# injun-baek/Video-Depth-Normal-v2

Hardware: AMD Instinct MI355X
Metric: depth frames/sec at 518x518, ViT-L (higher is better)
Workload: dtype f16x3; 1 GPU; DepthAnythingV2(vitl) batch=8 518x518 streams/GPU, memory bank full (S=6); replicas per GPU; lanes=2, precision=f16x3, ranks=1, backend=none, attention_pv_products=1

## Files before the change

video-depth-normal-v2_amd/csrc/attn.hip:

```cpp
#include "common.hpp"
#include <cstdlib>
#include <type_traits>
#include <utility>

namespace {

__device__ __forceinline__ bool lane_hi() { return (threadIdx.x & 32) != 0; }
__device__ __forceinline__ int perm23(int i) {
  return (i & ~12) | ((i & 4) << 1) | ((i & 8) >> 1);
}
__device__ __forceinline__ int acc_key(int reg, int h) {
  return (reg & 3) + 4 * ((reg >> 2) & 1) + 8 * h + 16 * (reg >> 3);
}

__device__ __forceinline__ float xhalf(float v) {
  const unsigned u = __builtin_bit_cast(unsigned, v);
  const auto r = __builtin_amdgcn_permlane32_swap(u, u, false, false);
  return __builtin_bit_cast(float, (lane_hi() ? r[0] : r[1]));
}

template <class F, int... J>
__device__ __forceinline__ void for_each_slot_impl(F& f, std::integer_sequence<int, J...>) {
  (f(std::integral_constant<int, J>{}), ...);
}
// ... 300 lines not shown
      for (int i = 0; i < 16; ++i) { o[0][i] *= alpha; o[1][i] *= alpha; }
    }
    if constexpr (VDN_ATTN_ABL & 2) asm volatile("s_waitcnt vmcnt(0) lgkmcnt(0)" ::: "memory");
    else stage_barrier();
  };

  stage_k(0, 0);
  if (nt > 1) stage_k(1, 1);
  stage_barrier();
  qk(0, s);
  stage_barrier();
  constexpr std::true_type Y{};
  constexpr std::false_type N{};
  if (nt == 1) {
    iter(0, N, N);
  } else {
    iter(0, N, Y);
    for (int t = 1; t + 1 < nt; ++t) iter(t, Y, Y);
    iter(nt - 1, Y, N);
  }
  pv((nt - 1) & 1, pf, pl);

  const float l_tot = l_run + __shfl_xor(l_run, 32);
  const float inv = 1.0f / l_tot;
  const int q = q0 + r;
  if (q < nq) {
    const int b = bh / H, hd = bh - b * H;
    const size_t oo = (((size_t)b * nq + q) * H + hd) * 64;
#pragma unroll
    for (int db = 0; db < 2; ++db)
#pragma unroll
      for (int g = 0; g < 4; ++g) {
        typename HT::V4 v, vl;
#pragma unroll
        for (int e = 0; e < 4; ++e) {
          const float x = o[db][4 * g + e] * inv;
          if (outl) {
            T a, b2;
            split_rtz(x, a, b2);
            v[e] = a;
            vl[e] = b2;
          } else {
            v[e] = (T)x;
          }
        }
        *(typename HT::V4*)(out + oo + db * 32 + 8 * g + 4 * h) = v;
        if (outl) *(typename HT::V4*)(outl + oo + db * 32 + 8 * g + 4 * h) = vl;
      }
  }
}

#include "attn2_kernel.hpp"

template <int DT, bool SPLIT, int NB >
__global__ __launch_bounds__(256) void temporal_attn_kernel(const typename Half<DT>::T* __restrict__ qkv,
                                                            typename Half<DT>::T* __restrict__ out,
                                                            const typename Half<DT>::T* __restrict__ qkv_lo,
                                                            typename Half<DT>::T* __restrict__ out_lo, int nseq,
                                                            int Tn, int D, int c, int heads, float scale_log2,
                                                            const float* __restrict__ rope_cs) {
  using HT = Half<DT>;
  using T = typename HT::T;
  using V8 = typename HT::V8;
  const int lane = threadIdx.x & 63;
  const int seq = blockIdx.x * 4 + (threadIdx.x >> 6);
  if (seq >= nseq) return;
  const int head = seq % heads;
  const int bd = seq / heads;
  const int d = bd % D, b = bd / D;
  const int dh = c / heads;
  const int r = lane & 31, h = lane >> 5;
  const size_t rs = (size_t)D * 3 * c;
  const size_t boff = ((size_t)b * Tn * D + d) * 3 * c + head * dh;
  const T* base = qkv + boff;
  const T* base_lo = SPLIT ? qkv_lo + boff : nullptr;
  const T* vb = base + 2 * c;
  const T* vb_lo = SPLIT ? base_lo + 2 * c : nullptr;
  const size_t ooff = ((size_t)b * Tn * D + d) * c + head * dh;
  T* ob = out + ooff;
  T* ob_lo = SPLIT ? out_lo + ooff : nullptr;
  const size_t os = (size_t)D * c;
  const int nks = (dh + 15) >> 4;
  const int neb = (dh + 31) >> 5;
  const int pk = perm23(r);

  for (int qb = 0; qb < NB; ++qb) {
    if (qb * 32 >= Tn) break;
    const int tq = qb * 32 + r;
    const int fq = tq < Tn ? tq : Tn - 1;
    f32x16 s[NB];
#pragma unroll
    for (int kb = 0; kb < NB; ++kb) {
#pragma unroll
      for (int i = 0; i < 16; ++i) s[kb][i] = 0.f;
      if (kb * 32 >= Tn) continue;
      const int tk = kb * 32 + pk;
      const int fk = tk < Tn ? tk : Tn - 1;
      for (int ks = 0; ks < nks; ++ks) {
        const int e0 = 16 * ks + 8 * h;
        V8 a, bq, al, bl;
#pragma unroll
        for (int j = 0; j < 8; ++j) { a[j] = (T)0.f; bq[j] = (T)0.f; al[j] = (T)0.f; bl[j] = (T)0.f; }
        if (e0 < dh) {
          bq = *(const V8*)(base + fq * rs + e0);
          a = *(const V8*)(base + fk * rs + c + e0);
          if constexpr (SPLIT) {
            bl = *(const V8*)(base_lo + fq * rs + e0);
            al = *(const V8*)(base_lo + fk * rs + c + e0);
          }
          if (rope_cs) {
            const size_t pair0 = (size_t)(head * dh + e0) >> 1;
            auto rot = [&](V8& hi, V8& lo, int frame) {
              const float* cs = rope_cs + ((size_t)frame * (c >> 1) + pair0) * 2;
#pragma unroll
              for (int j = 0; j < 8; j += 2) {
                const float x0 = (float)hi[j] + (SPLIT ? (float)lo[j] : 0.f), x1 = (float)hi[j + 1] + (SPLIT ? (float)lo[j + 1] : 0.f);
                const float cc = cs[j], ss = cs[j + 1];
                const float y0 = x0 * cc - x1 * ss, y1 = x0 * ss + x1 * cc;
                if constexpr (SPLIT) {
                  T h0, h1, l0, l1;
                  split2_rtz(y0, y1, h0, h1, l0, l1);
                  hi[j] = h0; hi[j + 1] = h1; lo[j] = l0; lo[j + 1] = l1;
                } else {
                  hi[j] = (T)y0; hi[j + 1] = (T)y1;
                }
              }
            };
            rot(bq, bl, fq);
            rot(a, al, fk);
          }
        }
        s[kb] = HT::mfma32(a, bq, s[kb]);
        if constexpr (SPLIT) {
          s[kb] = HT::mfma32(a, bl, s[kb]);
          s[kb] = HT::mfma32(al, bq, s[kb]);
        }
      }
    }
    float mx = -1e30f;
#pragma unroll
    for (int kb = 0; kb < NB; ++kb)
#pragma unroll
      for (int i = 0; i < 16; ++i) {
        float v = s[kb][i] * scale_log2;
        v = (kb * 32 + acc_key(i, h) < Tn) ? v : -INFINITY;
        s[kb][i] = v;
        mx = fmaxf(mx, v);
      }
    mx = fmaxf(mx, __shfl_xor(mx, 32));
    float ls = 0.f;
    V8 pf[NB][2], pl[NB][2];
#pragma unroll
    for (int kb = 0; kb < NB; ++kb)
#pragma unroll
      for (int i = 0; i < 16; ++i) {
        const float pv = __builtin_amdgcn_exp2f(s[kb][i] - mx);
        ls += pv;
        if constexpr (SPLIT) {
          T a2, b2;
          split_rtz(pv, a2, b2);
          pf[kb][i >> 3][i & 7] = a2;
          pl[kb][i >> 3][i & 7] = b2;
        } else {
          pf[kb][i >> 3][i & 7] = (T)pv;
        }
      }
    ls += __shfl_xor(ls, 32);
    const float inv = 1.0f / ls;

    for (int eb = 0; eb < neb; ++eb) {
      f32x16 o;
#pragma unroll
      for (int i = 0; i < 16; ++i) o[i] = 0.f;
      const int e = eb * 32 + r;
#pragma unroll
      for (int kb = 0; kb < NB; ++kb) {
        if (kb * 32 >= Tn) continue;
#pragma unroll
        for (int sp = 0; sp < 2; ++sp) {
          V8 a, al;
#pragma unroll
          for (int j = 0; j < 8; ++j) {
            const int key = kb * 32 + 16 * sp + 8 * h + j;
            const bool ok = key < Tn && e < dh;
            a[j] = ok ? vb[key * rs + e] : (T)0.f;
            if constexpr (SPLIT) al[j] = ok ? vb_lo[key * rs + e] : (T)0.f;
          }
          o = HT::mfma32(a, pf[kb][sp], o);
          if constexpr (SPLIT) {
            o = HT::mfma32(a, pl[kb][sp], o);
            o = HT::mfma32(al, pf[kb][sp], o);
          }
        }
      }
      if (tq < Tn) {
#pragma unroll
        for (int g = 0; g < 4; ++g) {
          const int e0 = eb * 32 + 8 * g + 4 * h;
          if (e0 < dh) {
            typename HT::V4 v, vl;
#pragma unroll
            for (int q = 0; q < 4; ++q) {
              const float x = o[4 * g + q] * inv;
              if constexpr (SPLIT) {
                T a2, b2;
                split_rtz(x, a2, b2);
                v[q] = a2;
                vl[q] = b2;
              } else {
                v[q] = (T)x;
              }
            }
            *(typename HT::V4*)(ob + tq * os + e0) = v;
            if constexpr (SPLIT) *(typename HT::V4*)(ob_lo + tq * os + e0) = vl;
          }
        }
      }
    }
  }
}

struct SlotTable { int s[32]; };

template <int DT, int CPL >
__global__ __launch_bounds__(256) void temporal_last_kernel(const float* __restrict__ pool, size_t slot_stride, SlotTable tab,
                                                            int T, int HW, int c,
                                                            const float* __restrict__ peq, const float* __restrict__ pek,
                                                            const float* __restrict__ pev, float scale,
                                                            typename Half<DT>::T* __restrict__ out,
                                                            typename Half<DT>::T* __restrict__ out_lo) {
  using Th = typename Half<DT>::T;
  const int lane = threadIdx.x & 63;
  const int px = blockIdx.x * 4 + (threadIdx.x >> 6);
  if (px >= HW) return;
  const int ch = lane * CPL;
  const size_t row = (size_t)px * 3 * c;
  float q[CPL];
  {
    const float* qn = pool + (size_t)tab.s[T - 1] * slot_stride + row + ch;
#pragma unroll
    for (int e = 0; e < CPL; ++e) q[e] = (qn[e] + peq[(size_t)(T - 1) * c + ch + e]) * scale;
  }
  float sc[32];
  float mx = -INFINITY;
#pragma unroll
  for (int t = 0; t < 32; ++t) {
    sc[t] = -INFINITY;
    if (t < T) {
      const float* kt = pool + (size_t)tab.s[t] * slot_stride + row + c + ch;
      const float* pk = pek + (size_t)t * c + ch;
      float d = 0.f;
#pragma unroll
      for (int e = 0; e < CPL; ++e) d = fmaf(q[e], kt[e] + pk[e], d);
      d += __shfl_xor(d, 1);
      d += __shfl_xor(d, 2);
      d += __shfl_xor(d, 4);
      sc[t] = d;
      mx = fmaxf(mx, d);
    }
  }
  float den = 0.f;
#pragma unroll
  for (int t = 0; t < 32; ++t) {
    sc[t] = t < T ? __expf(sc[t] - mx) : 0.f;
    den += sc[t];
  }
  const float inv = 1.0f / den;
  float o[CPL];
#pragma unroll
  for (int e = 0; e < CPL; ++e) o[e] = 0.f;
#pragma unroll
  for (int t = 0; t < 32; ++t) {
    if (t < T) {
      const float* vt = pool + (size_t)tab.s[t] * slot_stride + row + 2 * c + ch;
      const float* pv = pev + (size_t)t * c + ch;
      const float p = sc[t] * inv;
#pragma unroll
      for (int e = 0; e < CPL; ++e) o[e] = fmaf(p, vt[e] + pv[e], o[e]);
    }
  }
#pragma unroll
  for (int e = 0; e < CPL; ++e) store_half(out, out_lo, (size_t)px * c + ch + e, o[e]);
}

template <int DT>
int flash_launch(const void* Q, const void* K, const void* Vt, void* out, const void* Ql, const void* Kl, const void* Vtl,
                 void* outl, const void* Q8, const void* K8, void* out8, int out_kt, int B, int H, int nq, int nq_pad, int nk, int nk_pad,
                 float sl2, int pv, hipStream_t s) {
  using T = typename Half<DT>::T;
  const dim3 grid(((nq + 127) / 128) * B * H);
  const bool pv3 = pv == 3;
  const uint8_t* q8 = (const uint8_t*)Q8;
  const uint8_t* k8 = (const uint8_t*)K8;
  if ((out8 || out_kt || (Ql && !outl)) && !(Ql && !pv3 && q8 && k8 && DT == VDN_F16)) return VDN_EUNSUPPORTED;
  if (Ql && pv3)
    hipLaunchKernelGGL((flash_attn_kernel<DT, true, false, false>), grid, dim3(256), 65536, s, (const T*)Q, (const T*)K, (const T*)Vt,
                       (T*)out, (const T*)Ql, (const T*)Kl, (const T*)Vtl, (T*)outl, q8, k8, H, nq, nq_pad, nk, nk_pad, sl2);
  else if (Ql && q8 && k8 && DT == VDN_F16) {
    if constexpr (DT == VDN_F16) {
#ifndef VDN_ATTN2_NW
#define VDN_ATTN2_NW 4
#endif
      constexpr int NW = VDN_ATTN2_NW;
      const dim3 grid2(((nq + 32 * NW - 1) / (32 * NW)) * B * H);
      if (pv == 1)
        hipLaunchKernelGGL((flash_attn2_kernel<1, NW>), grid2, dim3(64 * NW), (VDN_ATTN_ABL & 32) ? 98304 : 65536, s, (const T*)Q, (const T*)K, (const T*)Vt, (T*)out,
                           (const T*)Kl, (const T*)Vtl, (T*)outl, q8, k8, H, nq, nq_pad, nk, nk_pad, sl2, (uint8_t*)out8, out_kt, B * nq);
      else
        hipLaunchKernelGGL((flash_attn2_kernel<2, NW>), grid2, dim3(64 * NW), (VDN_ATTN_ABL & 32) ? 98304 : 65536, s, (const T*)Q, (const T*)K, (const T*)Vt, (T*)out,
                           (const T*)Kl, (const T*)Vtl, (T*)outl, q8, k8, H, nq, nq_pad, nk, nk_pad, sl2, (uint8_t*)out8, out_kt, B * nq);
    }
  } else if (Ql)
    hipLaunchKernelGGL((flash_attn_kernel<DT, true, true, false>), grid, dim3(256), 65536, s, (const T*)Q, (const T*)K, (const T*)Vt,
                       (T*)out, (const T*)Ql, (const T*)Kl, (const T*)Vtl, (T*)outl, q8, k8, H, nq, nq_pad, nk, nk_pad, sl2);
  else
    hipLaunchKernelGGL((flash_attn_kernel<DT, false, false, false>), grid, dim3(256), 32768, s, (const T*)Q, (const T*)K, (const T*)Vt,
                       (T*)out, (const T*)nullptr, (const T*)nullptr, (const T*)nullptr, (T*)outl, q8, k8, H, nq, nq_pad, nk,
                       nk_pad, sl2);
  VDN_CHECK_LAUNCH();
  return VDN_OK;
}

template <int DT>
int temporal_launch(const void* qkv, void* out, const void* qkv_lo, void* out_lo, int nseq, int T, int D, int c, int heads,
                    float sl2, const float* rope_cs, hipStream_t s) {
  using TT = typename Half<DT>::T;
  const dim3 grid((nseq + 3) / 4);
#define VDN_TA(SP, NB_)                                                                                          \
  hipLaunchKernelGGL((temporal_attn_kernel<DT, SP, NB_>), grid, dim3(256), 0, s, (const TT*)qkv, (TT*)out,       \
                     (const TT*)(SP ? qkv_lo : nullptr), (TT*)(SP ? out_lo : nullptr), nseq, T, D, c, heads, sl2, rope_cs)
  if (qkv_lo) {
    if (T <= 32) VDN_TA(true, 1); else VDN_TA(true, 2);
  } else {
    if (T <= 32) VDN_TA(false, 1); else VDN_TA(false, 2);
  }
#undef VDN_TA
  VDN_CHECK_LAUNCH();
  return VDN_OK;
}

}

extern "C" int vdn_flash_attn(int dt, const void* Q, const void* K, const void* Vt, void* out, const void* Q_lo,
                              const void* K_lo, const void* Vt_lo, void* out_lo, const void* Q8, const void* K8, void* out8,
                              int out_kt, int B, int H, int nq, int nq_pad, int nk, int nk_pad, float scale, int pv_products,
                              vdn_stream stream) {
  if (!Q || !K || !Vt || !out || B <= 0 || H <= 0 || nq <= 0 || nk <= 0) return VDN_EINVAL;
  if (pv_products < 0 || pv_products > 3) return VDN_EINVAL;
  const int pv = pv_products ? pv_products : 1;
  if (nq_pad < nq || nk_pad < nk || (nk_pad & 63)) return VDN_EALIGN;
  if (((uintptr_t)Q | (uintptr_t)K | (uintptr_t)Vt | (uintptr_t)out) & 15) return VDN_EALIGN;
  const int nlo = (Q_lo != nullptr) + (K_lo != nullptr) + (Vt_lo != nullptr);
  if (nlo != 0 && nlo != 3) return VDN_EINVAL;
  if (nlo == 3 && !out_lo && !out8) return VDN_EINVAL;
  if (((uintptr_t)Q_lo | (uintptr_t)K_lo | (uintptr_t)Vt_lo | (uintptr_t)out_lo | (uintptr_t)Q8 | (uintptr_t)K8 | (uintptr_t)out8) & 15) return VDN_EALIGN;
  if ((Q8 == nullptr) != (K8 == nullptr) || (Q8 && (nlo != 3 || dt != VDN_F16))) return VDN_EINVAL;
  const float sl2 = scale * 1.44269504088896340736f;
  hipStream_t s = (hipStream_t)stream;
  if (dt == VDN_F16)
    return flash_launch<VDN_F16>(Q, K, Vt, out, Q_lo, K_lo, Vt_lo, out_lo, Q8, K8, out8, out_kt, B, H, nq, nq_pad, nk, nk_pad, sl2, pv, s);
  if (dt == VDN_BF16)
    return flash_launch<VDN_BF16>(Q, K, Vt, out, Q_lo, K_lo, Vt_lo, out_lo, nullptr, nullptr, out8, out_kt, B, H, nq, nq_pad, nk, nk_pad, sl2, pv, s);
  return VDN_EUNSUPPORTED;
}

extern "C" int vdn_temporal_attn(int dt, const void* qkv, void* out, const void* qkv_lo, void* out_lo, int Bv, int T,
                                 int D, int c, int heads, float scale, const float* rope_cs, vdn_stream stream) {
  if (!qkv || !out || Bv <= 0 || T <= 0 || T > 64 || D <= 0 || heads <= 0 || c % heads) return VDN_EINVAL;
  if ((qkv_lo == nullptr) != (out_lo == nullptr)) return VDN_EINVAL;
  const int dh = c / heads;
  if ((dh & 7) || dh > 256 || (c & 7)) return VDN_EALIGN;
  if (((uintptr_t)qkv | (uintptr_t)out | (uintptr_t)qkv_lo | (uintptr_t)out_lo) & 15) return VDN_EALIGN;
  const int nseq = Bv * D * heads;
  const float sl2 = scale * 1.44269504088896340736f;
  hipStream_t s = (hipStream_t)stream;
  return with_half(dt, [&](auto t) {
    return temporal_launch<decltype(t)::value>(qkv, out, qkv_lo, out_lo, nseq, T, D, c, heads, sl2, rope_cs, s);
  });
}

extern "C" int vdn_temporal_attn_last(int dt, const float* pool, size_t slot_stride, const int32_t* slots, int T, int HW,
                                      int c, const float* pe_q, const float* pe_k, const float* pe_v, float scale,
                                      void* out, void* out_lo, vdn_stream stream) {
  if (!pool || !slots || !pe_q || !pe_k || !pe_v || !out || T < 1 || T > 32 || HW <= 0) return VDN_EINVAL;
  if (slot_stride < (size_t)HW * 3 * c) return VDN_EINVAL;
  SlotTable tab;
  for (int t = 0; t < 32; ++t) {
    tab.s[t] = t < T ? slots[t] : 0;
    if (tab.s[t] < 0) return VDN_EINVAL;
  }
  if (c <= 0 || (c & 63) || c > 1024) return VDN_EUNSUPPORTED;
  hipStream_t s = (hipStream_t)stream;
  const dim3 grid((HW + 3) / 4), block(256);
#define VDN_TL(CPL_)                                                                                                     \
  hipLaunchKernelGGL((temporal_last_kernel<DT, CPL_>), grid, block, 0, s, pool, slot_stride, tab, T, HW, c, pe_q, pe_k, \
                     pe_v, scale, (typename Half<DT>::T*)out, (typename Half<DT>::T*)out_lo)
  return with_half(dt, [&](auto t) -> int {
    constexpr int DT = decltype(t)::value;
    switch (c) {
      case 64: VDN_TL(1); break;
      case 128: VDN_TL(2); break;
      case 192: VDN_TL(3); break;
      case 256: VDN_TL(4); break;
      case 384: VDN_TL(6); break;
      case 512: VDN_TL(8); break;
      case 768: VDN_TL(12); break;
      case 1024: VDN_TL(16); break;
      default: return VDN_EUNSUPPORTED;
    }
    VDN_CHECK_LAUNCH();
    return VDN_OK;
  });
#undef VDN_TL
}
```

video-depth-normal-v2_amd/csrc/attn2_kernel.hpp:

```cpp

template <int PV, int NW>
__global__ __launch_bounds__(64 * NW) __attribute__((amdgpu_waves_per_eu(2, 2))) void flash_attn2_kernel(
    const _Float16* __restrict__ Q, const _Float16* __restrict__ K, const _Float16* __restrict__ Vt, _Float16* __restrict__ out,
    const _Float16* __restrict__ Kl, const _Float16* __restrict__ Vtl, _Float16* __restrict__ outl, const uint8_t* __restrict__ Q8,
    const uint8_t* __restrict__ K8, int H, int nq, int nq_pad, int nk, int nk_pad, float scale_log2, uint8_t* __restrict__ out8,
    int out_kt, int out_rows) {
  using HT = Half<VDN_F16>;
  using T = _Float16;
  using V8 = typename HT::V8;
  constexpr int TILE = 8192;
  constexpr int NT = 4;
  extern __shared__ __attribute__((aligned(16))) char smem[];

  const int tid = threadIdx.x, lane = tid & 63;
  const int wave = __builtin_amdgcn_readfirstlane(tid >> 6);
  constexpr int QB = 32 * NW;
  constexpr int NPC = 8 / NW;
  const int nqb = (nq + QB - 1) / QB;
  const int logical = xcd_remap(blockIdx.x, gridDim.x);
  const int bh = logical / nqb;
  const int q0 = (logical - bh * nqb) * QB + wave * 32;
  const int r = lane & 31, h = lane >> 5;

  V8 qf[4];
  i32x8 q8h, q8l;
  {
    int q = q0 + r;
    q = q < nq ? q : nq - 1;
    const size_t qo = ((size_t)bh * nq_pad + q) * 64 + 8 * h;
#pragma unroll
    for (int ks = 0; ks < 4; ++ks) qf[ks] = *(const V8*)(Q + qo + 16 * ks);
    const uint8_t* q8 = Q8 + ((size_t)bh * nq_pad + q) * 128 + 32 * h;
    const u32x4 a0 = *(const u32x4*)q8, a1 = *(const u32x4*)(q8 + 16), b0 = *(const u32x4*)(q8 + 64), b1 = *(const u32x4*)(q8 + 80);
#pragma unroll
    for (int e = 0; e < 4; ++e) { q8h[e] = (int)a0[e]; q8h[4 + e] = (int)a1[e]; q8l[e] = (int)b0[e]; q8l[4 + e] = (int)b1[e]; }
  }

  const int lr = lane >> 3;
  const unsigned k_bytes = (unsigned)nk_pad * 64 * sizeof(T);
  const auto rsrc = [&](const void* base) {
    return __builtin_amdgcn_make_buffer_rsrc((void*)((const char*)base + (size_t)bh * k_bytes), 0, (int)k_bytes, 0x00020000);
  };
  const __amdgpu_buffer_rsrc_t rK = rsrc(K), rV = rsrc(Vt), rK8 = rsrc(K8), rVl = rsrc(Vtl);
  int koff[2], voff[2];
#pragma unroll
  for (int i = 0; i < NPC; ++i) {
    const int row = (wave + 4 * i) * 8 + lr;
    const int c = (lane & 7) ^ ((row >> 1) & 7);
    koff[i] = (row * 64 + c * 8) * (int)sizeof(T);
    voff[i] = (row * nk_pad + c * 8) * (int)sizeof(T);
  }
#define A2_BLDS16(rs, voffset, soffset, dst) \
  __builtin_amdgcn_raw_ptr_buffer_load_lds(rs, (__attribute__((address_space(3))) void*)(dst), 16, voffset, soffset, 0, 0)
  auto stage_k_piece = [&](int buf, int t, int i, bool second) {
    A2_BLDS16(second ? rK8 : rK, koff[i], t * (64 * 64 * (int)sizeof(T)), smem + buf * NT * TILE + (second ? 2 * TILE : 0) + (wave + 4 * i) * 1024);
  };
  auto stage_v_piece = [&](int buf, int t, int i, bool second) {
    A2_BLDS16(second ? rVl : rV, voff[i], t * (64 * (int)sizeof(T)), smem + buf * NT * TILE + TILE + (second ? 2 * TILE : 0) + (wave + 4 * i) * 1024);
  };

  const int k_base = perm23(r) * 128 + ((h ^ ((perm23(r) >> 1) & 7)) << 4);
  const int v_base = r * 128 + ((h ^ ((r >> 1) & 7)) << 4);
  const int k8_base = perm23(r) * 128 + (((2 * h) ^ ((perm23(r) >> 1) & 7)) << 4);
  auto k_addr = [&](int kb, int ks) { return kb * 4096 + (k_base ^ (ks << 5)); };
  auto v_addr = [&](int db, int c) { return db * 4096 + (v_base ^ (c << 5)); };
  auto k8_read = [&](const char* sK, int kb, int lo) {
    const char* p = sK + 2 * TILE + kb * 4096;
    const u32x4 a0 = *(const u32x4*)(p + (k8_base ^ ((4 * lo) << 4))), a1 = *(const u32x4*)(p + (k8_base ^ ((4 * lo + 1) << 4)));
    i32x8 v;
#pragma unroll
    for (int e = 0; e < 4; ++e) { v[e] = (int)a0[e]; v[4 + e] = (int)a1[e]; }
    return v;
  };
  auto cross_hl = [&](const i32x8& k8, f32x16 c) {
    return __builtin_amdgcn_mfma_scale_f32_32x32x64_f8f6f4(k8, q8l, c, 1, 1, 0, 127, 0, VDN_LO8_E8M0);
  };
  auto cross_lh = [&](const i32x8& k8l, f32x16 c) {
    return __builtin_amdgcn_mfma_scale_f32_32x32x64_f8f6f4(k8l, q8h, c, 1, 1, 0, VDN_LO8_E8M0, 0, 127);
  };

  f32x16 o[2], s[2][2];
  V8 pf[2][2][2];
#pragma unroll
  for (int i = 0; i < 16; ++i) { o[0][i] = 0.f; o[1][i] = 0.f; }
  float m_run = -1e30f, l_run = 0.f;
  constexpr float LAZY = 6.0f;
  const int nt = (nk + 63) >> 6;
  const f32x16 zero16 = {0.f, 0.f, 0.f, 0.f, 0.f, 0.f, 0.f, 0.f, 0.f, 0.f, 0.f, 0.f, 0.f, 0.f, 0.f, 0.f};

#if VDN_ATTN_ABL & 64
  unsigned long long stamp_sum[5] = {0, 0, 0, 0, 0}, stamp_last = 0;
#endif
#define A2_IC(n) std::integral_constant<int, n> {}
#define A2_PIN(x) asm volatile("" : "+v"(x))
  auto iter = [&](int t, auto has_prev_c, auto has_next_c, auto par_c) {
    constexpr bool HAS_PREV = decltype(has_prev_c)::value, HAS_NEXT = decltype(has_next_c)::value;
    constexpr int PAR = decltype(par_c)::value;
    const char* sKn = smem + (PAR ^ 1) * NT * TILE;
    const char* sVp = smem + (PAR ^ 1) * NT * TILE + TILE;
    f32x16(&sc)[2] = s[PAR];
    f32x16(&sn)[2] = s[PAR ^ 1];
    if constexpr (!HAS_NEXT) {
      if ((t + 1) * 64 > nk) {
#pragma unroll
        for (int kb = 0; kb < 2; ++kb)
#pragma unroll
          for (int i = 0; i < 16; ++i)
            if (t * 64 + kb * 32 + acc_key(i, h) >= nk) sc[kb][i] = -INFINITY;
      }
    }
    V8 fr[8];
    i32x8 f8[2];
    float mx = -1e30f, alpha = 1.f, mb = 0.f, ls0 = 0.f, ls1 = 0.f;
    float ff[2][2] = {{0.f, 0.f}, {0.f, 0.f}}, fe[2][2] = {{0.f, 0.f}, {0.f, 0.f}};
    unsigned pw[16];
    bool bump = false;
    const int tk = t + 2 < nt ? t + 2 : nt - 1;

    auto ldv = [&](auto cc, auto dbc, auto wc, auto bc) {
      if constexpr (HAS_PREV) fr[decltype(bc)::value] = *(const V8*)(sVp + decltype(wc)::value * 2 * TILE + v_addr(decltype(dbc)::value, decltype(cc)::value));
    };
    auto ldk = [&](auto kbc, auto ksc, auto bc) {
      if constexpr (HAS_NEXT) fr[decltype(bc)::value] = *(const V8*)(sKn + k_addr(decltype(kbc)::value, decltype(ksc)::value));
    };
    auto ldk8 = [&](auto kbc, auto loc, auto bc) {
      if constexpr (HAS_NEXT) f8[decltype(bc)::value] = k8_read(sKn, decltype(kbc)::value, decltype(loc)::value);
    };
    auto mpv = [&](auto cc, auto dbc, auto bc) {
      constexpr int c = decltype(cc)::value, db = decltype(dbc)::value;
      if constexpr (HAS_PREV) o[db] = HT::mfma32(fr[decltype(bc)::value], pf[PAR ^ 1][c >> 1][c & 1], o[db]);
    };
    auto mqk = [&](auto kbc, auto ksc, auto bc, auto firstc) {
      constexpr int kb = decltype(kbc)::value;
      if constexpr (HAS_NEXT) sn[kb] = HT::mfma32(fr[decltype(bc)::value], qf[decltype(ksc)::value], decltype(firstc)::value ? zero16 : sn[kb]);
    };
    auto mqx = [&](auto kbc, auto loc, auto bc, auto firstc) {
      constexpr int kb = decltype(kbc)::value;
      if constexpr (HAS_NEXT) {
        if constexpr (decltype(loc)::value == 0) sn[kb] = cross_hl(f8[decltype(bc)::value], decltype(firstc)::value ? zero16 : sn[kb]);
        else sn[kb] = cross_lh(f8[decltype(bc)::value], decltype(firstc)::value ? zero16 : sn[kb]);
      }
    };
    auto vmax = [&](auto qc) {
      constexpr int kb = decltype(qc)::value >> 1, i = (decltype(qc)::value & 1) * 8;
      mx = fmaxf(fmaxf(mx, sc[kb][i]), sc[kb][i + 1]);
      mx = fmaxf(fmaxf(mx, sc[kb][i + 2]), sc[kb][i + 3]);
      mx = fmaxf(fmaxf(mx, sc[kb][i + 4]), sc[kb][i + 5]);
      mx = fmaxf(fmaxf(mx, sc[kb][i + 6]), sc[kb][i + 7]);
    };
    auto vxh = [&]() { mx = fmaxf(mx, xhalf(mx)); };
    auto vbp = [&]() {
      bump = __builtin_amdgcn_ballot_w64((mx - m_run) * scale_log2 > LAZY) != 0;
      const float m_new = bump ? fmaxf(m_run, mx) : m_run;
      alpha = __builtin_amdgcn_exp2f((m_run - m_new) * scale_log2);
      m_run = m_new;
      mb = -m_new * scale_log2;
    };
    auto vf = [&](auto pc) {
      constexpr int p = decltype(pc)::value, kb = p >> 3, i = (p & 7) * 2;
      if constexpr (VDN_ATTN_ABL & 128) {
        ff[p & 1][0] = sc[kb][i];
        ff[p & 1][1] = sc[kb][i + 1];
      } else {
        ff[p & 1][0] = fmaf(sc[kb][i], scale_log2, mb);
        ff[p & 1][1] = fmaf(sc[kb][i + 1], scale_log2, mb);
      }
    };
    auto vx = [&](auto pc) {
      constexpr int p = decltype(pc)::value;
      fe[p & 1][0] = __builtin_amdgcn_exp2f(ff[p & 1][0]);
      fe[p & 1][1] = __builtin_amdgcn_exp2f(ff[p & 1][1]);
    };
    auto vc = [&](auto pc) {
      constexpr int p = decltype(pc)::value, f = p >> 2;
      pw[p] = __builtin_bit_cast(unsigned, __builtin_amdgcn_cvt_pkrtz(fe[p & 1][0], fe[p & 1][1]));
      const f16x2 pp = __builtin_bit_cast(f16x2, pw[p]);
      if constexpr (p & 1) { ls1 = __builtin_amdgcn_fdot2(pp, f16x2{(_Float16)1.f, (_Float16)1.f}, ls1, false); A2_PIN(ls1); }
      else { ls0 = __builtin_amdgcn_fdot2(pp, f16x2{(_Float16)1.f, (_Float16)1.f}, ls0, false); A2_PIN(ls0); }
      if constexpr ((p & 3) == 3) {
        pf[PAR][f >> 1][f & 1] = __builtin_bit_cast(V8, u32x4{pw[4 * f], pw[4 * f + 1], pw[4 * f + 2], pw[4 * f + 3]});
        A2_PIN(pf[PAR][f >> 1][f & 1]);
      }
    };
    auto vlr = [&]() { l_run = l_run * alpha + (ls0 + ls1); A2_PIN(l_run); };
    auto dma = [&](auto ic) {
      constexpr int i = decltype(ic)::value;
      if constexpr (((i & 3) >> 1) < NPC) {
        if constexpr (i < 4) {
          if constexpr (PV == 2 || !(i & 1)) stage_v_piece(PAR, t, i >> 1, i & 1);
        } else if constexpr (HAS_NEXT) {
          stage_k_piece(PAR, tk, (i - 4) >> 1, i & 1);
        }
      }
    };
#if VDN_ATTN_ABL & 16
#define A2_LDV(c, db, w, b) A2_PIN(fr[b]);
#define A2_LDK(kb, ks, b) A2_PIN(fr[b]);
#define A2_LDK8(kb, lo, b) A2_PIN(f8[b]);
#else
#define A2_LDV(c, db, w, b) ldv(A2_IC(c), A2_IC(db), A2_IC(w), A2_IC(b));
#define A2_LDK(kb, ks, b) ldk(A2_IC(kb), A2_IC(ks), A2_IC(b));
#define A2_LDK8(kb, lo, b) ldk8(A2_IC(kb), A2_IC(lo), A2_IC(b));
#endif
#if VDN_ATTN_ABL & 8
#define A2_PV(c, db, b)
#define A2_QK(kb, ks, b, f)
#define A2_QX(kb, lo, b, f)
#else
#define A2_PV(c, db, b) mpv(A2_IC(c), A2_IC(db), A2_IC(b));
#define A2_QK(kb, ks, b, f) mqk(A2_IC(kb), A2_IC(ks), A2_IC(b), A2_IC(f));
#define A2_QX(kb, lo, b, f) mqx(A2_IC(kb), A2_IC(lo), A2_IC(b), A2_IC(f));
#endif
#if VDN_ATTN_ABL & 4
#define A2_MAX(q)
#define A2_XH()
#define A2_BP()
#define A2_F(p)
#define A2_X(p)
#define A2_C(p)
#define A2_LR()
#else
#define A2_MAX(q) vmax(A2_IC(q));
#define A2_XH() vxh();
#define A2_BP() vbp();
#define A2_F(p) vf(A2_IC(p));
#define A2_X(p) vx(A2_IC(p));
#define A2_C(p) vc(A2_IC(p));
#define A2_LR() vlr();
#endif
#if VDN_ATTN_ABL & 1
#define A2_DMA(i)
#else
#define A2_DMA(i) dma(A2_IC(i));
#endif
#define A2_FENCE() __builtin_amdgcn_sched_barrier(0);
#if VDN_ATTN_ABL & 64
#define A2_STAMP(i) { const unsigned long long now = __builtin_amdgcn_s_memtime(); if (i > 0) stamp_sum[i - 1] += now - stamp_last; stamp_last = now; }
#ifndef VDN_ATTN2_STAMPS_INC
#define VDN_ATTN2_STAMPS_INC "attn2_stream_stamps.inc"
#endif
#include VDN_ATTN2_STAMPS_INC
#undef A2_STAMP
#else
#ifndef VDN_ATTN2_INC
#define VDN_ATTN2_INC "attn2_stream.inc"
#endif
    if constexpr (PV == 1) {
#include "attn2_stream_pv1.inc"
    } else {
#include VDN_ATTN2_INC
    }
#endif
#undef A2_LDV
#undef A2_LDK
#undef A2_LDK8
#undef A2_PV
#undef A2_QK
#undef A2_QX
#undef A2_MAX
#undef A2_XH
#undef A2_BP
#undef A2_F
#undef A2_X
#undef A2_C
#undef A2_LR
#undef A2_DMA
#undef A2_FENCE

    if constexpr (HAS_NEXT) { A2_PIN(sn[0]); A2_PIN(sn[1]); }
    if (bump) {
      asm volatile("" ::: "memory");
#pragma unroll
      for (int i = 0; i < 16; ++i) { o[0][i] *= alpha; o[1][i] *= alpha; }
    }
    if constexpr (VDN_ATTN_ABL & 2) asm volatile("s_waitcnt vmcnt(0) lgkmcnt(0)" ::: "memory");
    else stage_barrier();
#if VDN_ATTN_ABL & 64
    { const unsigned long long now = __builtin_amdgcn_s_memtime(); stamp_sum[4] += now - stamp_last; stamp_last = now; }
#endif
  };

  auto stage_k_all = [&](int buf, int t) {
#pragma unroll
    for (int i = 0; i < NPC; ++i) { stage_k_piece(buf, t, i, false); stage_k_piece(buf, t, i, true); }
  };
  stage_k_all(0, 0);
  if (nt > 1) stage_k_all(1, 1);
  stage_barrier();
#pragma unroll
  for (int kb = 0; kb < 2; ++kb) {
    s[0][kb] = cross_hl(k8_read(smem, kb, 0), zero16);
    s[0][kb] = cross_lh(k8_read(smem, kb, 1), s[0][kb]);
#pragma unroll
    for (int ks = 0; ks < 4; ++ks) s[0][kb] = HT::mfma32(*(const V8*)(smem + k_addr(kb, ks)), qf[ks], s[0][kb]);
  }
  stage_barrier();
  constexpr std::true_type Y{};
  constexpr std::false_type N{};
  if (nt == 1) {
    iter(0, N, N, A2_IC(0));
  } else {
    iter(0, N, Y, A2_IC(0));
    int t = 1;
    for (; t + 2 < nt; t += 2) {
      iter(t, Y, Y, A2_IC(1));
      iter(t + 1, Y, Y, A2_IC(0));
    }
    if (t + 1 < nt) { iter(t, Y, Y, A2_IC(1)); ++t; }
    if (t & 1) iter(t, Y, N, A2_IC(1));
    else iter(t, Y, N, A2_IC(0));
  }
  {
    const char* sV = smem + ((nt - 1) & 1) * NT * TILE + TILE;
    auto pv_last = [&](const V8(&p)[2][2]) {
#pragma unroll
      for (int c = 0; c < 4; ++c)
#pragma unroll
        for (int db = 0; db < 2; ++db) {
          o[db] = HT::mfma32(*(const V8*)(sV + v_addr(db, c)), p[c >> 1][c & 1], o[db]);
          if constexpr (PV == 2) o[db] = HT::mfma32(*(const V8*)(sV + 2 * TILE + v_addr(db, c)), p[c >> 1][c & 1], o[db]);
        }
    };
    if ((nt - 1) & 1) pv_last(pf[1]);
    else pv_last(pf[0]);
  }

#if VDN_ATTN_ABL & 64
  if (blockIdx.x == 300 && tid == 0)
    for (int i = 0; i < 5; ++i) ((unsigned long long*)out)[i] = stamp_sum[i];
#endif
  const float l_tot = l_run + __shfl_xor(l_run, 32);
  const float inv = 1.0f / l_tot;
  const int q = q0 + r;
  if (q < nq) {
    const int b = bh / H, hd = bh - b * H;
    const size_t row = (size_t)b * nq + q;
    const size_t oo = (row * H + hd) * 64;
    [[maybe_unused]] f16x32 hv6, lv6;
#pragma unroll
    for (int db = 0; db < 2; ++db)
#pragma unroll
      for (int g = 0; g < 4; ++g) {
        typename HT::V4 v, vl;
        float f[4];
#pragma unroll
        for (int e = 0; e < 4; ++e) {
          T a, b2;
          f[e] = o[db][4 * g + e] * inv;
          split_rtz(f[e], a, b2);
          v[e] = a;
          vl[e] = b2;
        }
        const int c = db * 32 + 8 * g + 4 * h;
        const size_t od = out_kt ? ((size_t)(2 * hd + db) * out_rows + row) * 32 + 8 * g + 4 * h : oo + c;
        *(typename HT::V4*)(out + od) = v;
        if (outl) *(typename HT::V4*)(outl + od) = vl;
        if constexpr (std::is_same_v<T, _Float16>) {
#pragma unroll
          for (int e = 0; e < 4; ++e) { hv6[16 * db + 4 * g + e] = v[e]; lv6[16 * db + 4 * g + e] = vl[e]; }
        }
      }
    if constexpr (std::is_same_v<T, _Float16>) {
      if (out8) {
        const int sb = x6_scale_byte(hv6);
        uint8_t* d8 = out8 + (out_kt ? ((size_t)hd * out_rows + row) * 64 : oo) + 32 * h;
        x6_store_half(d8, hv6, sb);
        x6_store_half(d8 + (size_t)out_rows * H * 64, lv6, sb - 10);
      }
    }
  }
#undef A2_IC
#undef A2_PIN
#undef A2_BLDS16
}
```

Measured before the change: 286.7 frames/s.

## Add optional persistent flash-attn2 grid with half-tile and dead-wave skipping

Restructures the flash_attn2 kernel into a loop over logical blocks so an optional persistent grid (VDN_ATTN_PERSIST=1) can prefetch the next block's K tiles and Q while the current block finishes, hiding the per-block prologue. By default the grid stays one block per tile, but two new skip flags are on: waves whose query rows are all out of range only issue the DMA and barriers, and a last key tile at most half full skips the empty half of the softmax and PV MFMAs. Buffer descriptors now span all heads, with per-head offsets passed as soffset, so a 4 GB size guard is added. The added opacity asm, sched barriers and control flow may raise register pressure or disturb the existing instruction schedule.

```diff
diff --git a/video-depth-normal-v2_amd/csrc/attn.hip b/video-depth-normal-v2_amd/csrc/attn.hip
--- a/video-depth-normal-v2_amd/csrc/attn.hip
+++ b/video-depth-normal-v2_amd/csrc/attn.hip
@@ -626,13 +626,36 @@
 #define VDN_ATTN2_NW 4
 #endif
       constexpr int NW = VDN_ATTN2_NW;
-      const dim3 grid2(((nq + 32 * NW - 1) / (32 * NW)) * B * H);
-      if (pv == 1)
-        hipLaunchKernelGGL((flash_attn2_kernel<1, NW>), grid2, dim3(64 * NW), (VDN_ATTN_ABL & 32) ? 98304 : 65536, s, (const T*)Q, (const T*)K, (const T*)Vt, (T*)out,
-                           (const T*)Kl, (const T*)Vtl, (T*)outl, q8, k8, H, nq, nq_pad, nk, nk_pad, sl2, (uint8_t*)out8, out_kt, B * nq);
-      else
-        hipLaunchKernelGGL((flash_attn2_kernel<2, NW>), grid2, dim3(64 * NW), (VDN_ATTN_ABL & 32) ? 98304 : 65536, s, (const T*)Q, (const T*)K, (const T*)Vt, (T*)out,
-                           (const T*)Kl, (const T*)Vtl, (T*)outl, q8, k8, H, nq, nq_pad, nk, nk_pad, sl2, (uint8_t*)out8, out_kt, B * nq);
+      constexpr size_t lds = (VDN_ATTN_ABL & 32) ? 98304 : 65536;
+      const int nblk = ((nq + 32 * NW - 1) / (32 * NW)) * B * H;
+      if ((unsigned long long)B * H * nk_pad * 64 * sizeof(T) > 0xFFFFFFFFull) return VDN_EUNSUPPORTED;
+      const auto slots = [](auto kernel) {
+        int per_cu = 0, dev = 0;
+        hipDeviceProp_t prop;
+        if (hipOccupancyMaxActiveBlocksPerMultiprocessor(&per_cu, kernel, 64 * NW, lds) != hipSuccess || per_cu <= 0) per_cu = 2;
+        if (hipGetDevice(&dev) != hipSuccess || hipGetDeviceProperties(&prop, dev) != hipSuccess) return 256 * per_cu;
+        return (prop.multiProcessorCount * per_cu) & ~7;
+      };
+      const char* e = getenv("VDN_ATTN_PERSIST");
+      const bool persist = e && atoi(e) == 1, plain = e && atoi(e) == 0;
+      e = getenv("VDN_ATTN_SKIP");
+      const int flags = plain ? 0 : (e ? atoi(e) & 3 : 3);
+      int res = nblk;
+      if (persist) {
+        static const int slots1 = slots(flash_attn2_kernel<1, NW, true>), slots2 = slots(flash_attn2_kernel<2, NW, true>);
+        res = pv == 1 ? slots1 : slots2;
+      }
+      const dim3 grid2(res >= 8 && res < nblk ? res : nblk);
+#define VDN_FA2(PV_, P_)                                                                                                        \
+  hipLaunchKernelGGL((flash_attn2_kernel<PV_, NW, P_>), grid2, dim3(64 * NW), lds, s, (const T*)Q, (const T*)K, (const T*)Vt,   \
+                     (T*)out, (const T*)Kl, (const T*)Vtl, (T*)outl, q8, k8, H, nq, nq_pad, nk, nk_pad, sl2, (uint8_t*)out8,    \
+                     out_kt, B * nq, nblk, flags)
+      if (pv == 1) {
+        if (persist) VDN_FA2(1, true); else VDN_FA2(1, false);
+      } else {
+        if (persist) VDN_FA2(2, true); else VDN_FA2(2, false);
+      }
+#undef VDN_FA2
     }
   } else if (Ql)
     hipLaunchKernelGGL((flash_attn_kernel<DT, true, true, false>), grid, dim3(256), 65536, s, (const T*)Q, (const T*)K, (const T*)Vt,
diff --git a/video-depth-normal-v2_amd/csrc/attn2_kernel.hpp b/video-depth-normal-v2_amd/csrc/attn2_kernel.hpp
--- a/video-depth-normal-v2_amd/csrc/attn2_kernel.hpp
+++ b/video-depth-normal-v2_amd/csrc/attn2_kernel.hpp
@@ -1,10 +1,10 @@
 
-template <int PV, int NW>
+template <int PV, int NW, bool PERSIST>
 __global__ __launch_bounds__(64 * NW) __attribute__((amdgpu_waves_per_eu(2, 2))) void flash_attn2_kernel(
     const _Float16* __restrict__ Q, const _Float16* __restrict__ K, const _Float16* __restrict__ Vt, _Float16* __restrict__ out,
     const _Float16* __restrict__ Kl, const _Float16* __restrict__ Vtl, _Float16* __restrict__ outl, const uint8_t* __restrict__ Q8,
     const uint8_t* __restrict__ K8, int H, int nq, int nq_pad, int nk, int nk_pad, float scale_log2, uint8_t* __restrict__ out8,
-    int out_kt, int out_rows) {
+    int out_kt, int out_rows, int nblk, int flags) {
   using HT = Half<VDN_F16>;
   using T = _Float16;
   using V8 = typename HT::V8;
@@ -17,31 +17,48 @@
   constexpr int QB = 32 * NW;
   constexpr int NPC = 8 / NW;
   const int nqb = (nq + QB - 1) / QB;
-  const int logical = xcd_remap(blockIdx.x, gridDim.x);
-  const int bh = logical / nqb;
-  const int q0 = (logical - bh * nqb) * QB + wave * 32;
   const int r = lane & 31, h = lane >> 5;
+  auto lane_now = [&](int& r_, int& h_) {
+    int z = 0;
+    asm volatile("" : "+s"(z));
+    const int l = __builtin_amdgcn_mbcnt_hi(~0u, __builtin_amdgcn_mbcnt_lo(~0u, z));
+    r_ = l & 31;
+    h_ = l >> 5;
+  };
+  auto block_at = [&](int b, int& bh_, int& q0_) {
+    const int logical = xcd_remap(b, nblk);
+    bh_ = logical / nqb;
+    q0_ = (logical - bh_ * nqb) * QB + wave * 32;
+  };
+  const int G = gridDim.x;
+  int blk = blockIdx.x, bh, q0, bhn, q0n;
+  block_at(blk, bh, q0);
 
   V8 qf[4];
   i32x8 q8h, q8l;
-  {
-    int q = q0 + r;
+  auto load_q = [&](int bh_, int q0_) {
+    int r_b, h_b;
+    lane_now(r_b, h_b);
+    int q = q0_ + r_b;
     q = q < nq ? q : nq - 1;
-    const size_t qo = ((size_t)bh * nq_pad + q) * 64 + 8 * h;
+    const size_t qo = ((size_t)bh_ * nq_pad + q) * 64 + 8 * h_b;
 #pragma unroll
     for (int ks = 0; ks < 4; ++ks) qf[ks] = *(const V8*)(Q + qo + 16 * ks);
-    const uint8_t* q8 = Q8 + ((size_t)bh * nq_pad + q) * 128 + 32 * h;
+    const uint8_t* q8 = Q8 + ((size_t)bh_ * nq_pad + q) * 128 + 32 * h_b;
     const u32x4 a0 = *(const u32x4*)q8, a1 = *(const u32x4*)(q8 + 16), b0 = *(const u32x4*)(q8 + 64), b1 = *(const u32x4*)(q8 + 80);
 #pragma unroll
     for (int e = 0; e < 4; ++e) { q8h[e] = (int)a0[e]; q8h[4 + e] = (int)a1[e]; q8l[e] = (int)b0[e]; q8l[4 + e] = (int)b1[e]; }
-  }
+  };
+  load_q(bh, q0);
 
   const int lr = lane >> 3;
   const unsigned k_bytes = (unsigned)nk_pad * 64 * sizeof(T);
   const auto rsrc = [&](const void* base) {
-    return __builtin_amdgcn_make_buffer_rsrc((void*)((const char*)base + (size_t)bh * k_bytes), 0, (int)k_bytes, 0x00020000);
+    return __builtin_amdgcn_make_buffer_rsrc((void*)base, 0, (int)(k_bytes * (unsigned)(nblk / nqb)), 0x00020000);
   };
   const __amdgpu_buffer_rsrc_t rK = rsrc(K), rV = rsrc(Vt), rK8 = rsrc(K8), rVl = rsrc(Vtl);
+  int nk_b = nk, nt_b = (nk + 63) >> 6, wave_b = wave;
+#define A2_OPAQUE(x) asm volatile("" : "+s"(x))
   int koff[2], voff[2];
 #pragma unroll
   for (int i = 0; i < NPC; ++i) {
@@ -52,11 +69,12 @@
   }
 #define A2_BLDS16(rs, voffset, soffset, dst) \
   __builtin_amdgcn_raw_ptr_buffer_load_lds(rs, (__attribute__((address_space(3))) void*)(dst), 16, voffset, soffset, 0, 0)
-  auto stage_k_piece = [&](int buf, int t, int i, bool second) {
-    A2_BLDS16(second ? rK8 : rK, koff[i], t * (64 * 64 * (int)sizeof(T)), smem + buf * NT * TILE + (second ? 2 * TILE : 0) + (wave + 4 * i) * 1024);
+  auto stage_k_piece = [&](int buf, bool next, int t, int i, bool second) {
+    A2_BLDS16(second ? rK8 : rK, koff[i], (unsigned)(next ? bhn : bh) * k_bytes + (unsigned)t * (64 * 64 * (unsigned)sizeof(T)),
+              smem + buf * NT * TILE + (second ? 2 * TILE : 0) + (wave_b + 4 * i) * 1024);
   };
   auto stage_v_piece = [&](int buf, int t, int i, bool second) {
-    A2_BLDS16(second ? rVl : rV, voff[i], t * (64 * (int)sizeof(T)), smem + buf * NT * TILE + TILE + (second ? 2 * TILE : 0) + (wave + 4 * i) * 1024);
+    A2_BLDS16(second ? rVl : rV, voff[i], (unsigned)bh * k_bytes + (unsigned)t * (64 * (unsigned)sizeof(T)), smem + buf * NT * TILE + TILE + (second ? 2 * TILE : 0) + (wave_b + 4 * i) * 1024);
   };
 
   const int k_base = perm23(r) * 128 + ((h ^ ((perm23(r) >> 1) & 7)) << 4);
@@ -81,11 +99,10 @@
 
   f32x16 o[2], s[2][2];
   V8 pf[2][2][2];
-#pragma unroll
-  for (int i = 0; i < 16; ++i) { o[0][i] = 0.f; o[1][i] = 0.f; }
   float m_run = -1e30f, l_run = 0.f;
   constexpr float LAZY = 6.0f;
   const int nt = (nk + 63) >> 6;
+  const bool half = (flags & 2) && nk - (nt - 1) * 64 <= 32;
   const f32x16 zero16 = {0.f, 0.f, 0.f, 0.f, 0.f, 0.f, 0.f, 0.f, 0.f, 0.f, 0.f, 0.f, 0.f, 0.f, 0.f, 0.f};
 
 #if VDN_ATTN_ABL & 64
@@ -93,20 +110,26 @@
 #endif
 #define A2_IC(n) std::integral_constant<int, n> {}
 #define A2_PIN(x) asm volatile("" : "+v"(x))
-  auto iter = [&](int t, auto has_prev_c, auto has_next_c, auto par_c) {
-    constexpr bool HAS_PREV = decltype(has_prev_c)::value, HAS_NEXT = decltype(has_next_c)::value;
+#define A2_KILL(x) asm volatile("" : "=v"(x))
+  auto iter = [&](int t, auto has_prev_c, auto has_next_c, auto par_c, auto half_c) {
+    constexpr bool HAS_PREV = decltype(has_prev_c)::value, HAS_NEXT = decltype(has_next_c)::value, HALF = decltype(half_c)::value;
     constexpr int PAR = decltype(par_c)::value;
+    static_assert(!(HALF && HAS_NEXT), "only the last tile can be half empty");
+    if constexpr (HALF) { A2_KILL(pf[PAR][1][0]); A2_KILL(pf[PAR][1][1]); }
+    if constexpr (!HAS_NEXT) { A2_KILL(s[PAR ^ 1][0]); A2_KILL(s[PAR ^ 1][1]); }
     const char* sKn = smem + (PAR ^ 1) * NT * TILE;
     const char* sVp = smem + (PAR ^ 1) * NT * TILE + TILE;
     f32x16(&sc)[2] = s[PAR];
     f32x16(&sn)[2] = s[PAR ^ 1];
     if constexpr (!HAS_NEXT) {
-      if ((t + 1) * 64 > nk) {
-#pragma unroll
-        for (int kb = 0; kb < 2; ++kb)
+      if ((t + 1) * 64 > nk_b) {
+        int r_b, h_b;
+        lane_now(r_b, h_b);
+#pragma unroll
+        for (int kb = 0; kb < (HALF ? 1 : 2); ++kb)
 #pragma unroll
           for (int i = 0; i < 16; ++i)
-            if (t * 64 + kb * 32 + acc_key(i, h) >= nk) sc[kb][i] = -INFINITY;
+            if (t * 64 + kb * 32 + acc_key(i, h_b) >= nk_b) sc[kb][i] = -INFINITY;
       }
     }
     V8 fr[8];
@@ -115,7 +138,8 @@
     float ff[2][2] = {{0.f, 0.f}, {0.f, 0.f}}, fe[2][2] = {{0.f, 0.f}, {0.f, 0.f}};
     unsigned pw[16];
     bool bump = false;
-    const int tk = t + 2 < nt ? t + 2 : nt - 1;
+    const bool k_next = PERSIST && (!HAS_NEXT || t + 2 >= nt_b);
+    const int tk = k_next ? PAR : t + 2 < nt_b ? t + 2 : nt_b - 1;
 
     auto ldv = [&](auto cc, auto dbc, auto wc, auto bc) {
       if constexpr (HAS_PREV) fr[decltype(bc)::value] = *(const V8*)(sVp + decltype(wc)::value * 2 * TILE + v_addr(decltype(dbc)::value, decltype(cc)::value));
@@ -124,7 +148,10 @@
       if constexpr (HAS_NEXT) fr[decltype(bc)::value] = *(const V8*)(sKn + k_addr(decltype(kbc)::value, decltype(ksc)::value));
     };
     auto ldk8 = [&](auto kbc, auto loc, auto bc) {
-      if constexpr (HAS_NEXT) f8[decltype(bc)::value] = k8_read(sKn, decltype(kbc)::value, decltype(loc)::value);
+      if constexpr (HAS_NEXT) {
+        f8[decltype(bc)::value] = k8_read(sKn, decltype(kbc)::value, decltype(loc)::value);
+        __builtin_amdgcn_sched_barrier(0);
+      }
     };
     auto mpv = [&](auto cc, auto dbc, auto bc) {
       constexpr int c = decltype(cc)::value, db = decltype(dbc)::value;
@@ -143,6 +170,7 @@
     };
     auto vmax = [&](auto qc) {
       constexpr int kb = decltype(qc)::value >> 1, i = (decltype(qc)::value & 1) * 8;
+      if constexpr (HALF && kb == 1) return;
       mx = fmaxf(fmaxf(mx, sc[kb][i]), sc[kb][i + 1]);
       mx = fmaxf(fmaxf(mx, sc[kb][i + 2]), sc[kb][i + 3]);
       mx = fmaxf(fmaxf(mx, sc[kb][i + 4]), sc[kb][i + 5]);
@@ -158,6 +186,7 @@
     };
     auto vf = [&](auto pc) {
       constexpr int p = decltype(pc)::value, kb = p >> 3, i = (p & 7) * 2;
+      if constexpr (HALF && kb == 1) return;
       if constexpr (VDN_ATTN_ABL & 128) {
         ff[p & 1][0] = sc[kb][i];
         ff[p & 1][1] = sc[kb][i + 1];
@@ -168,11 +197,13 @@
     };
     auto vx = [&](auto pc) {
       constexpr int p = decltype(pc)::value;
+      if constexpr (HALF && p >= 8) return;
       fe[p & 1][0] = __builtin_amdgcn_exp2f(ff[p & 1][0]);
       fe[p & 1][1] = __builtin_amdgcn_exp2f(ff[p & 1][1]);
     };
     auto vc = [&](auto pc) {
       constexpr int p = decltype(pc)::value, f = p >> 2;
+      if constexpr (HALF && p >= 8) return;
       pw[p] = __builtin_bit_cast(unsigned, __builtin_amdgcn_cvt_pkrtz(fe[p & 1][0], fe[p & 1][1]));
       const f16x2 pp = __builtin_bit_cast(f16x2, pw[p]);
       if constexpr (p & 1) { ls1 = __builtin_amdgcn_fdot2(pp, f16x2{(_Float16)1.f, (_Float16)1.f}, ls1, false); A2_PIN(ls1); }
@@ -188,8 +219,8 @@
       if constexpr (((i & 3) >> 1) < NPC) {
         if constexpr (i < 4) {
           if constexpr (PV == 2 || !(i & 1)) stage_v_piece(PAR, t, i >> 1, i & 1);
-        } else if constexpr (HAS_NEXT) {
-          stage_k_piece(PAR, tk, (i - 4) >> 1, i & 1);
+        } else if constexpr (PERSIST || HAS_NEXT) {
+          stage_k_piece(PAR, k_next, tk, (i - 4) >> 1, i & 1);
         }
       }
     };
@@ -280,96 +311,166 @@
 #endif
   };
 
+  auto s0 = [&]() {
+#pragma unroll
+    for (int kb = 0; kb < 2; ++kb) {
+      if (kb == 1 && half && nt == 1) { A2_KILL(s[0][1]); continue; }
+      s[0][kb] = cross_hl(k8_read(smem, kb, 0), zero16);
+      s[0][kb] = cross_lh(k8_read(smem, kb, 1), s[0][kb]);
+#pragma unroll
+      for (int ks = 0; ks < 4; ++ks) s[0][kb] = HT::mfma32(*(const V8*)(smem + k_addr(kb, ks)), qf[ks], s[0][kb]);
+    }
+  };
+  auto pv_last = [&](const V8(&p)[2][2], auto half_c) {
+    const char* sV = smem + ((nt_b - 1) & 1) * NT * TILE + TILE;
+#pragma unroll
+    for (int c = 0; c < (decltype(half_c)::value ? 2 : 4); ++c)
+#pragma unroll
+      for (int db = 0; db < 2; ++db) {
+        o[db] = HT::mfma32(*(const V8*)(sV + v_addr(db, c)), p[c >> 1][c & 1], o[db]);
+        if constexpr (PV == 2) o[db] = HT::mfma32(*(const V8*)(sV + 2 * TILE + v_addr(db, c)), p[c >> 1][c & 1], o[db]);
+      }
+  };
+  auto dead_iters = [&](int t0, int t1) {
+    for (int t = t0; t < t1; ++t) {
+      const int buf = t & 1;
+      const bool k_next = PERSIST && t + 2 >= nt_b;
+      const int tk = k_next ? buf : t + 2 < nt_b ? t + 2 : nt_b - 1;
+#pragma unroll
+      for (int i = 0; i < NPC; ++i) {
+        stage_v_piece(buf, t, i, false);
+        if constexpr (PV == 2) stage_v_piece(buf, t, i, true);
+      }
+      if (PERSIST || t + 1 < nt_b) {
+#pragma unroll
+        for (int i = 0; i < NPC; ++i) {
+          stage_k_piece(buf, k_next, tk, i, false);
+          stage_k_piece(buf, k_next, tk, i, true);
+        }
+      }
+      stage_barrier();
+    }
+  };
+
   auto stage_k_all = [&](int buf, int t) {
 #pragma unroll
-    for (int i = 0; i < NPC; ++i) { stage_k_piece(buf, t, i, false); stage_k_piece(buf, t, i, true); }
+    for (int i = 0; i < NPC; ++i) { stage_k_piece(buf, false, t, i, false); stage_k_piece(buf, false, t, i, true); }
   };
   stage_k_all(0, 0);
   if (nt > 1) stage_k_all(1, 1);
   stage_barrier();
-#pragma unroll
-  for (int kb = 0; kb < 2; ++kb) {
-    s[0][kb] = cross_hl(k8_read(smem, kb, 0), zero16);
-    s[0][kb] = cross_lh(k8_read(smem, kb, 1), s[0][kb]);
-#pragma unroll
-    for (int ks = 0; ks < 4; ++ks) s[0][kb] = HT::mfma32(*(const V8*)(smem + k_addr(kb, ks)), qf[ks], s[0][kb]);
-  }
-  stage_barrier();
+  bool dead = (flags & 1) && q0 >= nq;
+  if (!dead) s0();
   constexpr std::true_type Y{};
   constexpr std::false_type N{};
-  if (nt == 1) {
-    iter(0, N, N, A2_IC(0));
-  } else {
-    iter(0, N, Y, A2_IC(0));
-    int t = 1;
-    for (; t + 2 < nt; t += 2) {
-      iter(t, Y, Y, A2_IC(1));
-      iter(t + 1, Y, Y, A2_IC(0));
-    }
-    if (t + 1 < nt) { iter(t, Y, Y, A2_IC(1)); ++t; }
-    if (t & 1) iter(t, Y, N, A2_IC(1));
-    else iter(t, Y, N, A2_IC(0));
-  }
-  {
-    const char* sV = smem + ((nt - 1) & 1) * NT * TILE + TILE;
-    auto pv_last = [&](const V8(&p)[2][2]) {
-#pragma unroll
-      for (int c = 0; c < 4; ++c)
-#pragma unroll
-        for (int db = 0; db < 2; ++db) {
-          o[db] = HT::mfma32(*(const V8*)(sV + v_addr(db, c)), p[c >> 1][c & 1], o[db]);
-          if constexpr (PV == 2) o[db] = HT::mfma32(*(const V8*)(sV + 2 * TILE + v_addr(db, c)), p[c >> 1][c & 1], o[db]);
+  for (;;) {
+    const bool has_next = PERSIST && blk + G < nblk;
+    A2_OPAQUE(nk_b);
+    A2_OPAQUE(nt_b);
+    A2_OPAQUE(wave_b);
+    block_at(has_next ? blk + G : blk, bhn, q0n);
+    const bool dead_next = (flags & 1) && q0n >= nq;
+    asm volatile("s_waitcnt lgkmcnt(0)" ::: "memory");
+    __builtin_amdgcn_s_barrier();
+    asm volatile("" ::: "memory");
+    auto seam_s0 = [&]() {
+      A2_KILL(s[0][0]);
+      A2_KILL(s[0][1]);
+      A2_KILL(s[1][0]);
+      A2_KILL(s[1][1]);
+      if (has_next && !dead_next) s0();
+    };
+    if (dead) {
+      dead_iters(0, nt_b - 1);
+      if constexpr (PERSIST) load_q(bhn, q0n);
+      dead_iters(nt_b - 1, nt_b);
+      seam_s0();
+    } else {
+#pragma unroll
+      for (int i = 0; i < 16; ++i) { o[0][i] = 0.f; o[1][i] = 0.f; }
+      m_run = -1e30f;
+      l_run = 0.f;
+      A2_KILL(s[1][0]);
+      A2_KILL(s[1][1]);
+#pragma unroll
+      for (int i = 0; i < 8; ++i) A2_KILL(pf[i >> 2][(i >> 1) & 1][i & 1]);
+      if (nt_b > 1) {
+        iter(0, N, Y, A2_IC(0), N);
+        int t = 1;
+        for (; t + 2 < nt_b; t += 2) {
+          iter(t, Y, Y, A2_IC(1), N);
+          iter(t + 1, Y, Y, A2_IC(0), N);
         }
-    };
-    if ((nt - 1) & 1) pv_last(pf[1]);
-    else pv_last(pf[0]);
-  }
-
+        if (t + 1 < nt_b) iter(t, Y, Y, A2_IC(1), N);
+      }
+      if constexpr (PERSIST) load_q(bhn, q0n);
+      const int t = nt_b - 1;
+      auto last = [&](auto has_prev_c, auto par_c) {
+        if (half) iter(t, has_prev_c, N, par_c, Y);
+        else iter(t, has_prev_c, N, par_c, N);
+      };
+      if (t == 0) last(N, A2_IC(0));
+      else if (t & 1) last(Y, A2_IC(1));
+      else last(Y, A2_IC(0));
+      seam_s0();
+      if ((nt_b - 1) & 1) { if (half) pv_last(pf[1], Y); else pv_last(pf[1], N); }
+      else { if (half) pv_last(pf[0], Y); else pv_last(pf[0], N); }
 #if VDN_ATTN_ABL & 64
-  if (blockIdx.x == 300 && tid == 0)
-    for (int i = 0; i < 5; ++i) ((unsigned long long*)out)[i] = stamp_sum[i];
-#endif
-  const float l_tot = l_run + __shfl_xor(l_run, 32);
-  const float inv = 1.0f / l_tot;
-  const int q = q0 + r;
-  if (q < nq) {
-    const int b = bh / H, hd = bh - b * H;
-    const size_t row = (size_t)b * nq + q;
-    const size_t oo = (row * H + hd) * 64;
-    [[maybe_unused]] f16x32 hv6, lv6;
-#pragma unroll
-    for (int db = 0; db < 2; ++db)
-#pragma unroll
-      for (int g = 0; g < 4; ++g) {
-        typename HT::V4 v, vl;
-        float f[4];
-#pragma unroll
-        for (int e = 0; e < 4; ++e) {
-          T a, b2;
-          f[e] = o[db][4 * g + e] * inv;
-          split_rtz(f[e], a, b2);
-          v[e] = a;
-          vl[e] = b2;
+      if (blk == 300 && tid == 0)
+        for (int i = 0; i < 5; ++i) ((unsigned long long*)out)[i] = stamp_sum[i];
+#endif
+      const float l_tot = l_run + __shfl_xor(l_run, 32);
+      const float inv = 1.0f / l_tot;
+      int r_b, h_b;
+      lane_now(r_b, h_b);
+      const int q = q0 + r_b;
+      if (q < nq) {
+        const int b = bh / H, hd = bh - b * H;
+        const size_t row = (size_t)b * nq + q;
+        const size_t oo = (row * H + hd) * 64;
+        [[maybe_unused]] f16x32 hv6, lv6;
+#pragma unroll
+        for (int db = 0; db < 2; ++db)
+#pragma unroll
+          for (int g = 0; g < 4; ++g) {
+            typename HT::V4 v, vl;
+            float f[4];
+#pragma unroll
+            for (int e = 0; e < 4; ++e) {
+              T a, b2;
+              f[e] = o[db][4 * g + e] * inv;
+              split_rtz(f[e], a, b2);
+              v[e] = a;
+              vl[e] = b2;
+            }
+            const int c = db * 32 + 8 * g + 4 * h_b;
+            const size_t od = out_kt ? ((size_t)(2 * hd + db) * out_rows + row) * 32 + 8 * g + 4 * h_b : oo + c;
+            *(typename HT::V4*)(out + od) = v;
+            if (outl) *(typename HT::V4*)(outl + od) = vl;
+            if constexpr (std::is_same_v<T, _Float16>) {
+#pragma unroll
+              for (int e = 0; e < 4; ++e) { hv6[16 * db + 4 * g + e] = v[e]; lv6[16 * db + 4 * g + e] = vl[e]; }
+            }
+          }
+        if constexpr (std::is_same_v<T, _Float16>) {
+          if (out8) {
+            const int sb = x6_scale_byte(hv6);
+            uint8_t* d8 = out8 + (out_kt ? ((size_t)hd * out_rows + row) * 64 : oo) + 32 * h_b;
+            x6_store_half(d8, hv6, sb);
+            x6_store_half(d8 + (size_t)out_rows * H * 64, lv6, sb - 10);
+          }
         }
-        const int c = db * 32 + 8 * g + 4 * h;
-        const size_t od = out_kt ? ((size_t)(2 * hd + db) * out_rows + row) * 32 + 8 * g + 4 * h : oo + c;
-        *(typename HT::V4*)(out + od) = v;
-        if (outl) *(typename HT::V4*)(outl + od) = vl;
-        if constexpr (std::is_same_v<T, _Float16>) {
-#pragma unroll
-          for (int e = 0; e < 4; ++e) { hv6[16 * db + 4 * g + e] = v[e]; lv6[16 * db + 4 * g + e] = vl[e]; }
-        }
-      }
-    if constexpr (std::is_same_v<T, _Float16>) {
-      if (out8) {
-        const int sb = x6_scale_byte(hv6);
-        uint8_t* d8 = out8 + (out_kt ? ((size_t)hd * out_rows + row) * 64 : oo) + 32 * h;
-        x6_store_half(d8, hv6, sb);
-        x6_store_half(d8 + (size_t)out_rows * H * 64, lv6, sb - 10);
-      }
-    }
+      }
+    }
+    if (!has_next) break;
+    blk += G;
+    bh = bhn;
+    q0 = q0n;
+    dead = dead_next;
   }
 #undef A2_IC
 #undef A2_PIN
+#undef A2_KILL
+#undef A2_OPAQUE
 #undef A2_BLDS16
 }
```

Result: no change. 287.5 frames/s, median of 4 (+0.3%).
